# noveens/reviews4rec

Measured on AMD Instinct MI355X. Metric: train ratings/sec, higher is better.
Workload: dtype f32

## Files before the change

### include/r4r.h

```cpp
#ifndef R4R_H
#define R4R_H

#include <stddef.h>
#include <stdint.h>

#ifdef __cplusplus
extern "C" {
#endif

#define R4R_OK 0
#define R4R_ERR_ARG (-1)
#define R4R_ERR_LAUNCH (-2)
#define R4R_ERR_WORKSPACE (-3)

int r4r_version(void);
const char *r4r_last_error(void);

size_t r4r_textcnn_ws_bytes(int64_t N, int T, int E, int F, int64_t V);
int r4r_textcnn_fwd(const float *table, int64_t V, const int64_t *idx,
                    const float *conv_w, const float *conv_b,
                    float *pooled, int32_t *argmax,
                    void *ws, size_t ws_bytes,
                    int64_t N, int T, int E, int F, void *stream);

// ... 64 lines not shown
                       int64_t N, int R, int L, void *stream);

int r4r_mse_fwd_bwd(const float *out, const float *y, float *se, float *g_out,
                    int64_t N, float denom, void *stream);

int r4r_sqdist_mean_fwd(const float *a, const float *b, float *out, int64_t N, int L, void *stream);
int r4r_sqdist_mean_bwd(const float *a, const float *b, const float *g_out, float *g_a, float *g_b,
                        int64_t N, int L, void *stream);

int r4r_adam_chunk_elems(void);
int r4r_adam_multi(int ntensor, const uint64_t *p, const uint64_t *g, const uint64_t *m, const uint64_t *v,
                   const int64_t *numel, float lr, double beta1, double beta2, float eps,
                   float weight_decay, int64_t step, const int64_t *step_dev, void *stream);
int r4r_adam_gathered(float *p, const float *gathered, int world, float *g_sum, float *m, float *v,
                      int64_t numel, float lr, double beta1, double beta2, float eps,
                      float weight_decay, int64_t step, void *stream);
int r4r_adam_gathered_guarded(float *p, const float *gathered, int world, float *g_sum, float *m, float *v,
                              int64_t numel, float lr, double beta1, double beta2, float eps,
                              float weight_decay, int64_t step, const uint32_t *abort_word, void *stream);

int r4r_peer_segment_create(int64_t bytes, void **ptr, uint8_t *handle);
int r4r_peer_segment_open(const uint8_t *handle, void **ptr);
int r4r_peer_segment_close(void *ptr);
int r4r_peer_segment_destroy(void *ptr);
int r4r_peer_push(const float *src, int64_t numel, const uint64_t *peer_dst, const uint64_t *peer_flags,
                  uint32_t *arrive, int rank, int world, uint32_t epoch, const uint32_t *wait_flags,
                  uint32_t *timed_out, double timeout_s, void *stream);
int r4r_peer_wait(const uint32_t *flags, int world, uint32_t epoch, uint32_t *timed_out, double timeout_s, void *stream);


#define R4R_CONV_AUTO 0
#define R4R_CONV_DIRECT 1
#define R4R_CONV_PROJECT 2
int r4r_deepconn_nparam(void);
int r4r_deepconn_layout(int E, int L, int64_t *offsets, int64_t *sizes, int64_t *total);
size_t r4r_deepconn_ws_bytes(int64_t B, int T, int E, int L, int64_t V);
size_t r4r_deepconn_ws_mult_offset(int64_t B, int T, int E, int L, int64_t V);
size_t r4r_deepconn_ws_count_offset(int64_t B, int T, int E, int L, int64_t V, int tower, int buffer);
size_t r4r_deepconn_ws_partials_offset(int64_t B, int T, int E, int L, int64_t V, int tower, int which);
size_t r4r_deepconn_ws_plan_offset(int64_t B, int T, int E, int L, int64_t V, int tower, int buffer, int which);
size_t r4r_deepconn_ws_state_offset(int64_t B, int T, int E, int L, int64_t V, int tower, int buffer, int which);
int r4r_deepconn_step(const float *table, int64_t V, const int64_t *user_idx, const int64_t *item_idx,
                      const float *y, float *flat_p, float *flat_g,
                      float *pred, float *se, float *sse_accum,
                      void *ws, size_t ws_bytes,
                      int64_t B, int T, int E, int L,
                      float dropout_p, int training, uint64_t seed, uint64_t offset,
                      float inv_denom, int conv_algo, int token_buffer, int tokens_ready,
                      const int64_t *next_user_idx, const int64_t *next_item_idx,
                      float *flat_m, float *flat_v, float lr, double beta1, double beta2, float eps,
                      float weight_decay, int64_t adam_step, void *stream);
int r4r_deepconn_tail_fold(int on);
int r4r_deepconn_tail(int64_t B, int E, int L);
int r4r_deepconn_tokens(const int64_t *user_idx, const int64_t *item_idx, void *ws, size_t ws_bytes,
                        int64_t B, int T, int E, int L, int64_t V, int conv_algo, int token_buffer,
                        int discard, void *stream);

#define R4R_TIMING_TEXTCNN_FWD 0
#define R4R_TIMING_TEXTCNN_WGRAD 1
#define R4R_TIMING_ADAM 2
#define R4R_TIMING_PROJ_GEMM 3
#define R4R_TIMING_PROJ_GATHER 4
#define R4R_TIMING_SLOTS 8
int r4r_timing_enable(int slot_mask);
int r4r_timing_read(int slot, double *total_ms, int64_t *count, int reset);

size_t r4r_mf_ws_bytes(int64_t B, int D, int64_t n_users, int64_t n_items);
size_t r4r_mf_ws_persist_bytes(int64_t B, int D, int64_t n_users, int64_t n_items);
size_t r4r_mf_ws_mult_offset(int64_t B, int D, int64_t n_users, int64_t n_items);
size_t r4r_mf_ws_grad_offset(int64_t B, int D, int64_t n_users, int64_t n_items, int which);
int r4r_mf_step(const int64_t *uid, const int64_t *iid, const float *y,
                const uint64_t *p, const uint64_t *m, const uint64_t *v,
                int64_t n_users, int64_t n_items, int D,
                float *pred, float *se, float *sse_accum, void *ws, size_t ws_bytes, int64_t B,
                float dropout_p, int training, uint64_t seed, uint64_t offset, float inv_denom,
                int sweep_period, int64_t sweep_base, int sweep_all,
                float lr, double beta1, double beta2, float eps, float weight_decay, int64_t adam_step,
                void *stream);

int r4r_mf_rows_flush(const uint64_t *p, const uint64_t *m, const uint64_t *v,
                      int64_t n_users, int64_t n_items, int D, void *ws, size_t ws_bytes, int64_t B,
                      int sweep_period, int64_t sweep_base,
                      float lr, double beta1, double beta2, float eps, float weight_decay, int64_t adam_step,
                      void *stream);
size_t r4r_mf_ws_flag_offset(int64_t B, int D, int64_t n_users, int64_t n_items);

int r4r_sse_accumulate(const float *se, int64_t n, float *accum, void *stream);

size_t r4r_mf_dp_block_bytes(int64_t B_pad, int D);
int r4r_mf_grad(const int64_t *uid, const int64_t *iid, const float *y, const uint64_t *p,
                const uint64_t *m, const uint64_t *v,
                int64_t n_users, int64_t n_items, int D, float *pred, float *se, void *block, float *mult,
                int64_t B, int64_t B_pad, float dropout_p, int training, uint64_t seed, uint64_t offset,
                float inv_denom, void *ws, int sweep_period, int64_t sweep_base,
                float lr, double beta1, double beta2, float eps, float weight_decay, int64_t adam_step,
                void *stream);
int r4r_mf_apply(const void *blocks, int world, int64_t B_pad, const uint64_t *p, const uint64_t *m,
                 const uint64_t *v, int64_t n_users, int64_t n_items, int D, void *ws, size_t ws_bytes,
                 int sweep_period, int64_t sweep_base, int sweep_all,
                 const float *se, int64_t se_n, float *sse_accum,
                 float lr, double beta1, double beta2, float eps, float weight_decay, int64_t adam_step,
                 void *stream);
int r4r_mf_grad_push(const int64_t *uid, const int64_t *iid, const float *y, const uint64_t *p,
                     const uint64_t *m, const uint64_t *v,
                     int64_t n_users, int64_t n_items, int D, float *pred, float *se, float *mult,
                     int64_t B, int64_t B_pad, float dropout_p, int training, uint64_t seed, uint64_t offset,
// ... 390 lines not shown
```

### reviews4rec_amd/csrc/engine.hip

```cpp
#include <stdlib.h>

#include "trace_device.h"
#include "textcnn.h"
#include "wgrad_device.h"
#include "tokens_device.h"
#include "adam_device.h"

namespace r4r {

constexpr int F_CONV = 100;
constexpr int FM_K = 8;
constexpr int MAX_L = 128;

enum { P_UCW = 0, P_UCB, P_UFW, P_UFB, P_ICW, P_ICB, P_IFW, P_IFB, P_FMV, P_FMLW, P_FMLB, P_GB, P_COUNT };

struct Layout {
    int64_t off[P_COUNT], size[P_COUNT], total;
};

static Layout make_layout(int E, int L) {
    Layout lay;
    const int64_t sz[P_COUNT] = {(int64_t)F_CONV * 3 * E, F_CONV, (int64_t)L * F_CONV, L,
                                 (int64_t)F_CONV * 3 * E, F_CONV, (int64_t)L * F_CONV, L,
                                 (int64_t)2 * L * FM_K, 2 * L, 1, 1};
    int64_t o = 0;
    for (int i = 0; i < P_COUNT; ++i) {
        lay.off[i] = o;
        lay.size[i] = sz[i];
        o += (sz[i] + 31) & ~(int64_t)31;
    }
    lay.total = o;
    return lay;
}

struct HeadArgs {
    const float *pmax[2]; const int *parg[2];
    const float *fc_w[2]; const float *fc_b[2];
    const float *V, *lin_w, *lin_b, *gbias;
    const float *y;
    float *pooled[2]; int *argmax[2];
    float *g_pooled[2];
    float *mult;
    float *x, *s, *g, *gz;
    float *pred, *se;
    int64_t B;
    int L, tiles, training, want_grad;
    float p_drop, inv_denom;
    uint64_t seed, offset;
    PlanArgs plan;
    int *plan_spent[2];
    TokenArgs marks;
    int mark_wgs;
};


constexpr int HEAD_MAX_TILES = 8;

#define SEL2(arr, s) ((s) ? (arr)[1] : (arr)[0])
HEAD_TRACE_DEFINE(r4r_debug_dc_head_trace)
template <int ML>
__global__ __launch_bounds__(256) void deepconn_head_wg_kernel(HeadArgs a) {
    if ((int64_t)blockIdx.x >= a.B) {
        const int fb = (int)blockIdx.x - (int)a.B, flag_wgs = (2 * a.plan.units + 3) / 4;
        if (fb < flag_wgs) {
            segment_flags_wave(a.plan, fb * 4 + (int)(threadIdx.x >> 6));
        } else {
            const HeadArgs &A = kernel_args<HeadArgs>();
            token_mark_block(A.marks, fb - flag_wgs, A.mark_wgs, 256);
        }
        return;
    }
    HEAD_STAMP(0)
    constexpr int N2 = 2 * ML, PARTS = 256 / N2;
    __shared__ float sw[2][ML][F_CONV + 1];
    __shared__ float sfb[N2], slw[N2], sz[N2];
    __shared__ float sV[N2][FM_K];
    __shared__ float sp[2][F_CONV + 4];
    __shared__ float red[N2][PARTS + 1];
    const int tid = threadIdx.x, lane = tid & 63, w = tid >> 6;
    const int64_t b = blockIdx.x;
    const int L = a.L, n = 2 * L;
    const float lin_b0 = a.lin_b[0], gbias0 = a.gbias[0], yb = a.y ? a.y[b] : 0.f;

    constexpr int FQ = F_CONV / 4;
    typedef float hq4 __attribute__((ext_vector_type(4)));
    constexpr int WREGS = (2 * ML * FQ + 255) / 256;
    hq4 wreg[WREGS];
    const int wtot = 2 * L * FQ;
#pragma unroll
    for (int k = 0; k < WREGS; ++k) {
        const int i = min(tid + 256 * k, wtot - 1);
        const int t = i >= L * FQ;
        wreg[k] = *reinterpret_cast<const hq4 *>(SEL2(a.fc_w, t) + 4 * (i - t * L * FQ));
    }
    const int tn = min(tid, n - 1);
    const float fbreg = SEL2(a.fc_b, tn >= L)[tn - (tn >= L ? L : 0)];
    const float lwreg = a.lin_w[tn];
    constexpr int VREGS = (N2 * FM_K + 255) / 256;
    float vreg[VREGS];
#pragma unroll
    for (int k = 0; k < VREGS; ++k) vreg[k] = a.V[min(tid + 256 * k, n * FM_K - 1)];
    if (b == 0 && tid < 2 && SEL2(a.plan_spent, tid)) SEL2(a.plan_spent, tid)[0] = 0;

    {
        const int t = w >> 1, f = lane + 64 * (w & 1), fc = min(f, F_CONV - 1);
        float best = -INFINITY;
        int bp = -1;
        if (a.tiles <= HEAD_MAX_TILES) {
            float v[HEAD_MAX_TILES];
            int pp[HEAD_MAX_TILES];
#pragma unroll
            for (int k = 0; k < HEAD_MAX_TILES; ++k) {
                const size_t o = ((size_t)b * a.tiles + min(k, a.tiles - 1)) * NP + fc;
                v[k] = SEL2(a.pmax, t)[o];
                pp[k] = SEL2(a.parg, t)[o];
            }
#pragma unroll
            for (int k = 0; k < HEAD_MAX_TILES; ++k)
                if (v[k] > best) { best = v[k]; bp = pp[k]; }
        } else {
            for (int k0 = 0; k0 < a.tiles; k0 += HEAD_MAX_TILES) {
                float v[HEAD_MAX_TILES];
                int pp[HEAD_MAX_TILES];
#pragma unroll
                for (int k = 0; k < HEAD_MAX_TILES; ++k) {
                    const bool in = k0 + k < a.tiles;
                    const size_t o = ((size_t)b * a.tiles + (in ? k0 + k : 0)) * NP + fc;
                    v[k] = in ? SEL2(a.pmax, t)[o] : -INFINITY;
                    pp[k] = SEL2(a.parg, t)[o];
                }
#pragma unroll
                for (int k = 0; k < HEAD_MAX_TILES; ++k)
                    if (v[k] > best) { best = v[k]; bp = pp[k]; }
            }
        }
        if (!(best > 0.f)) { best = 0.f; bp = -1; }
        if (f < F_CONV) {
            sp[t][f] = best;
            SEL2(a.pooled, t)[b * F_CONV + f] = best;
            SEL2(a.argmax, t)[b * F_CONV + f] = bp;
        }
    }
    HEAD_STAMP(1)
#pragma unroll
    for (int k = 0; k < WREGS; ++k) {
        const int i = tid + 256 * k;
        if (i < wtot) {
            const int t = i >= L * FQ, r = i - t * L * FQ, l = r / FQ, f0 = 4 * (r - l * FQ);
#pragma unroll
            for (int c = 0; c < 4; ++c) sw[t][l][f0 + c] = wreg[k][c];
        }
    }
    if (tid < n) { sfb[tid] = fbreg; slw[tid] = lwreg; }
#pragma unroll
    for (int k = 0; k < VREGS; ++k) {
        const int i = tid + 256 * k;
        if (i < n * FM_K) sV[i / FM_K][i % FM_K] = vreg[k];
    }
    __syncthreads();
    HEAD_STAMP(2)

    {
        const int o = tid / PARTS, part = tid - o * PARTS;
        if (o < n) {
            const int t = o / L, l = o - t * L;
            float acc = 0.f;
            for (int f = part; f < F_CONV; f += PARTS) acc = fmaf(sp[t][f], sw[t][l][f], acc);
            red[o][part] = acc;
        }
    }
    __syncthreads();
    const bool has_y = a.y != nullptr, want = has_y && a.want_grad;
    if (w == 0) {
        constexpr int NI = (N2 + 63) / 64;
        float xi[NI], mult[NI], lw[NI], gacc[NI];
#pragma unroll
        for (int u = 0; u < NI; ++u) {
            const int i = lane + 64 * u;
            xi[u] = 0.f; mult[u] = 1.f; gacc[u] = 0.f;
            lw[u] = (i < n) ? slw[i] : 0.f;
            if (i < n) {
                float acc = 0.f;
#pragma unroll
                for (int q = 0; q < PARTS; ++q) acc += red[i][q];
                xi[u] = acc + sfb[i];
            }
            if (a.training && a.p_drop > 0.f && i < n) {
                const uint32_t r = philox_first_word(a.offset + (uint64_t)(b * n + i), a.seed);
                const float uu = (float)(r >> 8) * (1.0f / 16777216.0f);
                mult[u] = (uu >= a.p_drop) ? 1.f / (1.f - a.p_drop) : 0.f;
            }
            xi[u] *= mult[u];
        }
        float inter = 0.f;
        float sk_keep[FM_K];
#pragma unroll
        for (int k = 0; k < FM_K; ++k) {
            float pv = 0.f, pv2 = 0.f, vv[NI];
#pragma unroll
            for (int u = 0; u < NI; ++u) {
                const int i = lane + 64 * u;
                vv[u] = (i < n) ? sV[i][k] : 0.f;
                pv += xi[u] * vv[u];
                pv2 += xi[u] * xi[u] * vv[u] * vv[u];
            }
            const float sk = wave_sum(pv);
            const float s2 = wave_sum(pv2);
            inter += sk * sk - s2;
#pragma unroll
            for (int u = 0; u < NI; ++u) gacc[u] += sk * vv[u] - xi[u] * vv[u] * vv[u];
            sk_keep[k] = sk;
        }
        float pl = 0.f;
#pragma unroll
        for (int u = 0; u < NI; ++u) pl += xi[u] * lw[u];
        const float lin = wave_sum(pl);
        const float pred = (0.5f * inter + lin + lin_b0) + gbias0;
        if (lane == 0) a.pred[b] = pred;
        if (has_y) {
            const float d = pred - yb;
            if (lane == 0) a.se[b] = d * d;
            if (want) {
                const float g = 2.f * d * a.inv_denom;
#pragma unroll
                for (int u = 0; u < NI; ++u) {
                    const int i = lane + 64 * u;
                    const float gx = g * (gacc[u] + lw[u]);
                    const float gz = gx * mult[u];
                    if (i < n) {
                        sz[i] = gz;
                        a.x[b * n + i] = xi[u];
                        a.gz[b * n + i] = gz;
                        a.mult[b * n + i] = mult[u];
                    }
                }
                if (lane < FM_K) {
                    float sv = 0.f;
#pragma unroll
                    for (int k = 0; k < FM_K; ++k) if (lane == k) sv = sk_keep[k];
                    a.s[b * FM_K + lane] = sv;
                }
                if (lane == 0) a.g[b] = g;
            }
        }
    }
    if (!want) return;
    __syncthreads();
    HEAD_STAMP(3)
    if (tid < 2 * F_CONV) {
        const int t = tid >= F_CONV, f = tid - t * F_CONV;
        float acc = 0.f;
        for (int l = 0; l < L; ++l) acc = fmaf(sz[t * L + l], sw[t][l][f], acc);
        SEL2(a.g_pooled, t)[b * F_CONV + f] = acc;
    }
    HEAD_STAMP(4)
}

struct HeadGradArgs {
    const float *pooled[2];
    const float *x, *s, *g, *gz;
    const float *V;
    const float *se;
    float *g_fc_w[2], *g_fc_b[2], *g_V, *g_lin_w, *g_lin_b, *g_gb;
    float *sse_accum;
    int64_t B;
    int L;
};

constexpr int HG_ROWS = 16, HG_COLS = 16;
template <bool STEP = false>
__device__ __forceinline__ void head_grad_block(const HeadGradArgs &a, int blk, const FlatAdam *opt = nullptr) {
    __shared__ float red[HG_ROWS][HG_COLS];
    const int ox = threadIdx.x & (HG_COLS - 1), rg = threadIdx.x / HG_COLS;
    const int L = a.L, n = 2 * L;
    const int n_fcw = L * F_CONV;
    const int seg[9] = {n_fcw, L, n_fcw, L, n * FM_K, n, 1, 1, 1};
    int o = blk * HG_COLS + ox;
    int which = -1, local = 0, acc_o = o;
#pragma unroll
    for (int k = 0; k < 9; ++k) {
        if (which < 0) {
            if (acc_o < seg[k]) { which = k; local = acc_o; }
            else acc_o -= seg[k];
        }
    }
    float P = 0.f, M = 0.f, V = 0.f;
    int po = 0;
    bool stepping = false;
    if constexpr (STEP) {
        if (opt->on && rg == 0 && which >= 0 && which < 8) {
            const float *dst = which == 0 ? a.g_fc_w[0] + local : (which == 1 ? a.g_fc_b[0] + local : (which == 2 ? a.g_fc_w[1] + local :
                  (which == 3 ? a.g_fc_b[1] + local : (which == 4 ? a.g_V + local : (which == 5 ? a.g_lin_w + local :
                  (which == 6 ? a.g_lin_b : a.g_gb))))));
            po = (int)(dst - opt->g);
            stepping = true;
        }
    }
    float s = 0.f;
    if (which >= 0) {
        const bool is_w = which == 0 || which == 2, is_b = which == 1 || which == 3, is_v = which == 4, is_lw = which == 5;
        const int t = which >> 1;
        const int wl = local / F_CONV, wf = local - wl * F_CONV;
        const int vi = local / FM_K, vk = local - vi * FM_K;
        const float *pa = (is_w || is_b) ? a.gz : (which == 8 ? a.se : a.g);
        const int64_t sa = (is_w || is_b) ? n : 1;
        const int64_t oa = is_w ? t * L + wl : (is_b ? t * L + local : 0);
// ... 43 lines not shown
        }
        if constexpr (STEP) {
            if (stepping) {
                adam_elem(P, t, M, V, opt->s);
                opt->p[po] = P; opt->m[po] = M; opt->v[po] = V;
            }
        }
    }
}

BWD_TRACE_DEFINE(r4r_debug_dc_bwd_trace)
struct DcBackwardArgs {
    WgradArgs w;
    HeadGradArgs h;
    int hg_blocks;
    TokenArgs nx;
    PlanArgs plan;
};
__global__ __launch_bounds__(WG_THREADS, 8) void deepconn_backward_kernel(DcBackwardArgs) {
    const DcBackwardArgs &A = kernel_args<DcBackwardArgs>();
    const WgradArgs &w = A.w;
    const HeadGradArgs &h = A.h;
    const TokenArgs &nx = A.nx;
    const PlanArgs &plan = A.plan;
    const int hg_blocks = A.hg_blocks;
    BWD_STAMP(0, wall_clock64())
    BWD_STAMP(2, (unsigned long long)blockIdx.z + 1)
    if (blockIdx.z == 1 || blockIdx.z == 2) {
        wgrad_block(w, blockIdx.x, blockIdx.y, blockIdx.z - 1);
    } else if (blockIdx.z == 0) {
        for (int blk = blockIdx.y * gridDim.x + blockIdx.x; blk < hg_blocks; blk += gridDim.x * gridDim.y) {
            head_grad_block(h, blk);
            __syncthreads();
        }
    } else {
        const int np = plan.units > 0 ? 2 : 0, blk = blockIdx.y * gridDim.x + blockIdx.x;
        if (blk < np) segment_plan_block<WG_THREADS>(plan, blk);
        else token_mark_block(nx, blk - np, gridDim.x * gridDim.y - np, WG_THREADS);
    }
#ifdef R4R_TRACE
    __syncthreads();
#endif
    BWD_STAMP(1, wall_clock64())
}

struct DcFoldArgs {
    WgradArgs w;
    FlatAdam opt;
    HeadGradArgs h;
    int hg_blocks;
    TokenArgs nx;
    PlanArgs plan;
    int comp_blocks;
};
static_assert(WG_THREADS % 64 == 0, "the 256-thread roles of the fold launch are whole waves: the others end before any barrier");
template <bool BIGV>
__global__ __launch_bounds__(WG_ROW_MAX_THREADS, 8) void deepconn_backward_fold_kernel(DcFoldArgs) {
    const DcFoldArgs &A = kernel_args<DcFoldArgs>();
    BWD_STAMP(0, wall_clock64())
    BWD_STAMP(2, (unsigned long long)blockIdx.z + 1)
    if (blockIdx.z == 1 || blockIdx.z == 2) {
        wgrad_row_block(A.w, A.opt, blockIdx.x, blockIdx.y, blockIdx.z - 1);
    } else {
        if (threadIdx.x >= WG_THREADS) return;
        const int blk0 = blockIdx.y * gridDim.x + blockIdx.x, nblk = gridDim.x * gridDim.y;
        if (blockIdx.z == 0) {
            for (int blk = blk0; blk < A.hg_blocks; blk += nblk) {
                head_grad_block<true>(A.h, blk, &A.opt);
                __syncthreads();
            }
        } else {
            const int np = A.plan.units > 0 ? 2 : 0, comp_blocks = A.comp_blocks;
            const int blk = ((int)blockIdx.z - 3) * nblk + blk0;
            if (blk < np) {
                segment_plan_block<WG_THREADS>(A.plan, blk);
            } else if (blk - np < 2 * comp_blocks) {
                const int t = (blk - np) >= comp_blocks;
                const TokenTower &tw = t ? A.nx.t[1] : A.nx.t[0];
                if constexpr (BIGV) token_compact_block<WG_THREADS / 64, COMPACT_BIG_G>(tw, A.nx.V, blk - np - t * comp_blocks);
                else token_compact_block<WG_THREADS / 64, 1>(tw, A.nx.V, blk - np - t * comp_blocks);
            }
        }
    }
#ifdef R4R_TRACE
    __syncthreads();
#endif
    BWD_STAMP(1, wall_clock64())
}

constexpr int RED_THREADS = 256;
struct FusedAdam {
    float *p, *m, *v;
    const float *g;
    int64_t lo[2], hi[2];
    AdamScalars s;
    int on;
};
__global__ __launch_bounds__(RED_THREADS) void deepconn_reduce_kernel(WgradArgs w, int red_blocks, int comp_blocks,
                                                                      TokenArgs nx, FusedAdam opt) {
    const int bx = blockIdx.x;
    if (bx < red_blocks) {
        const WgradTower &tw = w.t[blockIdx.y];
        const int nw = w.F * 3 * w.E;
        const int i = bx * RED_THREADS + threadIdx.x;
        const float *gp0 = i < nw ? tw.d_w + i : (i < nw + w.F ? tw.d_b + (i - nw) : nullptr);
        const int64_t o = gp0 ? gp0 - opt.g : 0;
        float P = 0.f, M = 0.f, V = 0.f;
        if (opt.on && gp0) { P = opt.p[o]; M = opt.m[o]; V = opt.v[o]; }
        float *dst;
        const float g = wgrad_reduce_elem(w, blockIdx.y, i, dst);
        if (opt.on && dst) {
            adam_elem(P, g, M, V, opt.s);
            opt.p[o] = P; opt.m[o] = M; opt.v[o] = V;
        }
    } else if (bx < red_blocks + comp_blocks) {
        token_compact_auto<RED_THREADS / 64>(nx.t[blockIdx.y], nx.V, bx - red_blocks);
    } else {
        const int64_t o = opt.lo[blockIdx.y] + (int64_t)(bx - red_blocks - comp_blocks) * RED_THREADS + threadIdx.x;
        if (o < opt.hi[blockIdx.y]) {
            float P = opt.p[o], M = opt.m[o], V = opt.v[o];
            adam_elem(P, opt.g[o], M, V, opt.s);
            opt.p[o] = P; opt.m[o] = M; opt.v[o] = V;
        }
    }
}

__global__ void sse_only_kernel(const float *__restrict__ se, float *__restrict__ accum, int64_t B) {
    __shared__ float red[256];
    float s = 0.f;
    for (int64_t i = threadIdx.x; i < B; i += 256) s += se[i];
    red[threadIdx.x] = s;
    __syncthreads();
    for (int off = 128; off > 0; off >>= 1) {
        if ((int)threadIdx.x < off) red[threadIdx.x] += red[threadIdx.x + off];
        __syncthreads();
    }
    if (threadIdx.x == 0) accum[0] += red[0];
}

struct StepWs {
    float *wp[2], *pmax[2]; int *parg[2];
    int *flags[2][2], *slot[2][2], *list[2][2], *count[2][2]; float *ptab[2];
    int *live[2][2], *perm[2][2], *plan_ready[2][2];
    float *pooled[2]; int *argmax[2]; float *g_pooled[2];
    float *mult, *x, *s, *g, *gz;
    float *part_w[2], *part_b[2];
    size_t bytes;
};

static StepWs carve(void *ws, int64_t B, int T, int E, int L, int64_t V) {
    StepWs w;
    char *p = static_cast<char *>(ws);
    auto take = [&](size_t nbytes) { char *r = p; p += align256(nbytes); return r; };
    const size_t tiles128 = (size_t)(T + 2 + 127) / 128;
    const int ns = textcnn_wgrad_splits(B);
    for (int t = 0; t < 2; ++t) {
        w.wp[t] = reinterpret_cast<float *>(take(textcnn_wp_floats(E) * 4));
        w.pmax[t] = reinterpret_cast<float *>(take((size_t)B * tiles128 * NP * 4));
        w.parg[t] = reinterpret_cast<int *>(take((size_t)B * tiles128 * NP * 4));
        w.pooled[t] = reinterpret_cast<float *>(take((size_t)B * F_CONV * 4));
        w.argmax[t] = reinterpret_cast<int *>(take((size_t)B * F_CONV * 4));
        w.g_pooled[t] = reinterpret_cast<float *>(take((size_t)B * F_CONV * 4));
        w.part_w[t] = reinterpret_cast<float *>(take((size_t)ns * F_CONV * 3 * E * 4));
        w.part_b[t] = reinterpret_cast<float *>(take((size_t)ns * F_CONV * 4));
        for (int bf = 0; bf < 2; ++bf) {
            w.flags[bf][t] = reinterpret_cast<int *>(take((size_t)(V + 4) * 4));
            w.slot[bf][t] = reinterpret_cast<int *>(take((size_t)(V + 4) * 4));
            w.list[bf][t] = reinterpret_cast<int *>(take((size_t)proj_row_capacity(B, T, V) * 4));
            w.count[bf][t] = reinterpret_cast<int *>(take(256));
        }
        w.ptab[t] = reinterpret_cast<float *>(take(proj_ptab_floats(B, T, V) * 4));
    }
    w.mult = reinterpret_cast<float *>(take((size_t)B * 2 * L * 4));
    w.x = reinterpret_cast<float *>(take((size_t)B * 2 * L * 4));
    w.gz = reinterpret_cast<float *>(take((size_t)B * 2 * L * 4));
    w.s = reinterpret_cast<float *>(take((size_t)B * FM_K * 4));
    w.g = reinterpret_cast<float *>(take((size_t)B * 4));
    for (int t = 0; t < 2; ++t)
        for (int bf = 0; bf < 2; ++bf) {
            w.live[bf][t] = reinterpret_cast<int *>(take((size_t)PLAN_MAX_UNITS * 4));
            w.perm[bf][t] = reinterpret_cast<int *>(take((size_t)PLAN_MAX_UNITS * 4));
            w.plan_ready[bf][t] = reinterpret_cast<int *>(take(256));
        }
    w.bytes = (size_t)(p - static_cast<char *>(ws));
    return w;
}

}

using namespace r4r;

extern "C" int r4r_deepconn_nparam(void) { return P_COUNT; }

extern "C" int r4r_deepconn_layout(int E, int L, int64_t *offsets, int64_t *sizes, int64_t *total) {
    R4R_REQUIRE(E > 0 && L > 0 && L <= MAX_L && offsets && sizes && total, "deepconn_layout: bad arguments");
    const Layout lay = make_layout(E, L);
    for (int i = 0; i < P_COUNT; ++i) { offsets[i] = lay.off[i]; sizes[i] = lay.size[i]; }
    *total = lay.total;
    return R4R_OK;
}

extern "C" size_t r4r_deepconn_ws_bytes(int64_t B, int T, int E, int L, int64_t V) {
    if (B < 0 || T <= 0 || E <= 0 || L <= 0 || V <= 0) return 0;
    return carve(nullptr, B, T, E, L, V).bytes;
}

extern "C" size_t r4r_deepconn_ws_mult_offset(int64_t B, int T, int E, int L, int64_t V) {
    char base[1];
    const StepWs w = carve(base, B, T, E, L, V);
    return (size_t)(reinterpret_cast<char *>(w.mult) - base);
}

extern "C" size_t r4r_deepconn_ws_count_offset(int64_t B, int T, int E, int L, int64_t V, int tower, int buffer) {
    char base[1];
    const StepWs w = carve(base, B, T, E, L, V);
    return (size_t)(reinterpret_cast<char *>(w.count[buffer & 1][tower & 1]) - base);
}

extern "C" size_t r4r_deepconn_ws_partials_offset(int64_t B, int T, int E, int L, int64_t V, int tower, int which) {
    char base[1];
    const StepWs w = carve(base, B, T, E, L, V);
    const void *at = which ? static_cast<const void *>(w.parg[tower & 1]) : w.pmax[tower & 1];
    return (size_t)(static_cast<const char *>(at) - base);
}
extern "C" size_t r4r_deepconn_ws_plan_offset(int64_t B, int T, int E, int L, int64_t V, int tower, int buffer, int which) {
    char base[1];
    const StepWs w = carve(base, B, T, E, L, V);
    const int t = tower & 1, bf = buffer & 1;
    const void *at[3] = {w.perm[bf][t], w.plan_ready[bf][t], w.live[bf][t]};
    return (which < 0 || which > 2) ? 0 : (size_t)(static_cast<const char *>(at[which]) - base);
}

extern "C" size_t r4r_deepconn_ws_state_offset(int64_t B, int T, int E, int L, int64_t V, int tower, int buffer, int which) {
    char base[1];
    const StepWs w = carve(base, B, T, E, L, V);
    const int t = tower & 1, bf = buffer & 1;
    const void *at[4] = {w.flags[bf][t], w.slot[bf][t], w.list[bf][t], w.argmax[t]};
    return (which < 0 || which > 3) ? 0 : (size_t)(static_cast<const char *>(at[which]) - base);
}

static bool plan_applies(int64_t B, int T) {
    const int tiles = proj_tiles(T);
    return proj_gather_plan() && (tiles & 1) == 0 && B * tiles <= PLAN_MAX_UNITS;
}

static int g_tail_fold = -1;
static int tail_fold_switch() {
    if (g_tail_fold < 0) {
        const char *e = getenv("R4R_TAIL");
        g_tail_fold = (e && e[0] == 'o') ? 0 : 1;
    }
    return g_tail_fold;
}
static bool tail_folds(int64_t B, int E, int L) {
    if (!tail_fold_switch() || B < 1 || E <= 0 || E % 4 != 0 || L > 64) return false;
    const int ns = textcnn_wgrad_splits(B);
    return wgrad_row_applies(B, E, ns, (int)cdiv(B, ns));
}
extern "C" int r4r_deepconn_tail_fold(int on) {
    const int before = tail_fold_switch();
    g_tail_fold = on ? 1 : 0;
    return before;
}
extern "C" int r4r_deepconn_tail(int64_t B, int E, int L) { return tail_folds(B, E, L) ? 1 : 0; }

extern "C" int r4r_deepconn_tokens(const int64_t *user_idx, const int64_t *item_idx, void *ws, size_t ws_bytes,
                                   int64_t B, int T, int E, int L, int64_t V, int conv_algo, int token_buffer,
                                   int discard, void *stream) {
    R4R_REQUIRE(user_idx && item_idx && ws, "deepconn_tokens: null pointer");
    R4R_REQUIRE(token_buffer == 0 || token_buffer == 1, "deepconn_tokens: token_buffer must be 0 or 1");
    if (ws_bytes < r4r_deepconn_ws_bytes(B, T, E, L, V)) {
        set_error("deepconn_tokens: workspace %zu < %zu bytes", ws_bytes, r4r_deepconn_ws_bytes(B, T, E, L, V));
        return R4R_ERR_WORKSPACE;
    }
    if (B == 0 || textcnn_pick_algo(conv_algo, B, T, E, F_CONV) != R4R_CONV_PROJECT) return R4R_OK;
    const StepWs w = carve(ws, B, T, E, L, V);
    if (discard) {
        for (int t = 0; t < 2; ++t) {
            (void)hipMemsetAsync(w.count[token_buffer][t], 0, sizeof(int), as_stream(stream));
            (void)hipMemsetAsync(w.plan_ready[token_buffer][t], 0, sizeof(int), as_stream(stream));
        }
        return check_launch("deepconn_tokens(discard)");
    }
    ProjTower pt[2];
    const int64_t *idx[2] = {user_idx, item_idx};
    for (int t = 0; t < 2; ++t) {
        pt[t] = ProjTower{};
        pt[t].idx = idx[t];
        pt[t].flags = w.flags[token_buffer][t]; pt[t].slot = w.slot[token_buffer][t];
        pt[t].list = w.list[token_buffer][t]; pt[t].count = w.count[token_buffer][t];
    }
    return textcnn_proj_tokens_launch(V, pt, 2, B, T, false, as_stream(stream));
}

extern "C" int r4r_deepconn_step(const float *table, int64_t V, const int64_t *user_idx, const int64_t *item_idx,
                                 const float *y, float *flat_p, float *flat_g,
                                 float *pred, float *se, float *sse_accum,
                                 void *ws, size_t ws_bytes,
                                 int64_t B, int T, int E, int L,
                                 float dropout_p, int training, uint64_t seed, uint64_t offset,
                                 float inv_denom, int conv_algo, int token_buffer, int tokens_ready,
                                 const int64_t *next_user_idx, const int64_t *next_item_idx,
                                 float *flat_m, float *flat_v, float lr, double beta1, double beta2, float eps,
                                 float weight_decay, int64_t adam_step,
                                 void *stream) {
    R4R_REQUIRE(table && user_idx && item_idx && flat_p && pred && ws, "deepconn_step: null pointer");
    R4R_REQUIRE(!flat_m == !flat_v, "deepconn_step: flat_m and flat_v go together");
    R4R_REQUIRE(!flat_m || (flat_g && adam_step >= 1), "deepconn_step: the fused optimiser needs gradients and "
                                                       "adam_step >= 1");
    R4R_REQUIRE(!next_user_idx == !next_item_idx, "deepconn_step: next_user_idx and next_item_idx go together");
    R4R_REQUIRE(!next_user_idx || flat_g, "deepconn_step: the next batch's tokens ride on the backward launches "
                                          "(training steps only)");
    R4R_REQUIRE(V > 0 && B >= 0 && T > 0, "deepconn_step: bad sizes");
    R4R_REQUIRE(E > 0 && E % 4 == 0, "deepconn_step: word_embed_size %d must be a positive multiple of 4", E);
    R4R_REQUIRE(L > 0 && L <= MAX_L, "deepconn_step: latent_size %d outside 1..%d", L, MAX_L);
    R4R_REQUIRE(!flat_g || (y && se), "deepconn_step: gradients need ratings y and the se buffer");
    R4R_REQUIRE(!y || se, "deepconn_step: se buffer required when y is given");
// ... 38 lines not shown
    } else {
        FwdTower ft[2];
        for (int t = 0; t < 2; ++t) {
            ft[t].idx = idx[t];
            ft[t].conv_w = P[t ? P_ICW : P_UCW];
            ft[t].conv_b = P[t ? P_ICB : P_UCB];
            ft[t].wp = w.wp[t]; ft[t].pmax = w.pmax[t]; ft[t].parg = w.parg[t];
        }
        if (int rc = textcnn_fwd_launch(table, ft, 2, B, T, E, F_CONV, st)) return rc;
        tiles = textcnn_tiles(T);
    }

    HeadArgs h;
    for (int t = 0; t < 2; ++t) {
        h.pmax[t] = w.pmax[t]; h.parg[t] = w.parg[t];
        h.fc_w[t] = P[t ? P_IFW : P_UFW]; h.fc_b[t] = P[t ? P_IFB : P_UFB];
        h.pooled[t] = w.pooled[t]; h.argmax[t] = w.argmax[t]; h.g_pooled[t] = w.g_pooled[t];
    }
    h.V = P[P_FMV]; h.lin_w = P[P_FMLW]; h.lin_b = P[P_FMLB]; h.gbias = P[P_GB];
    h.y = y; h.mult = w.mult; h.x = w.x; h.s = w.s; h.g = w.g; h.gz = w.gz;
    h.pred = pred; h.se = se;
    h.B = B; h.L = L; h.tiles = tiles; h.training = training; h.want_grad = flat_g != nullptr;
    h.p_drop = dropout_p; h.inv_denom = inv_denom; h.seed = seed; h.offset = offset;
    const bool planning = next_user_idx && flat_g && algo == R4R_CONV_PROJECT && plan_applies(B, T);
    PlanArgs plan{};
    if (planning) {
        const int ob = token_buffer ^ 1;
        plan.idx[0] = next_user_idx; plan.idx[1] = next_item_idx;
        for (int t = 0; t < 2; ++t) {
            plan.live[t] = w.live[ob][t]; plan.perm[t] = w.perm[ob][t]; plan.plan_ready[t] = w.plan_ready[ob][t];
        }
        plan.T = T; plan.tiles = proj_tiles(T); plan.units = (int)(B * plan.tiles);
    }
    h.plan = plan;
    for (int t = 0; t < 2; ++t) h.plan_spent[t] = algo == R4R_CONV_PROJECT ? w.plan_ready[token_buffer][t] : nullptr;
    const bool fold = flat_g && tail_folds(B, E, L);
    const bool prefetch = next_user_idx && algo == R4R_CONV_PROJECT;
    TokenArgs nx{};
    if (prefetch) {
        ProjTower nt[2];
        const int64_t *nidx[2] = {next_user_idx, next_item_idx};
        const int ob = token_buffer ^ 1;
        for (int t = 0; t < 2; ++t) {
            nt[t] = ProjTower{};
            nt[t].idx = nidx[t];
            nt[t].flags = w.flags[ob][t]; nt[t].slot = w.slot[ob][t];
            nt[t].list = w.list[ob][t]; nt[t].count = w.count[ob][t];
        }
        nx = make_token_args(V, nt, 2, B, T);
    }
    h.marks = nx;
    const int64_t mark_want = cdiv(B * (int64_t)T, 256);
    h.mark_wgs = (fold && prefetch) ? (int)(mark_want < 1024 ? mark_want : 1024) : 0;
    const unsigned head_wgs = (unsigned)B + (unsigned)cdiv(2 * (int64_t)plan.units, 4) + (unsigned)h.mark_wgs;
    if (L <= 16) deepconn_head_wg_kernel<16><<<head_wgs, 256, 0, st>>>(h);
    else if (L <= 32) deepconn_head_wg_kernel<32><<<head_wgs, 256, 0, st>>>(h);
    else if (L <= 64) deepconn_head_wg_kernel<64><<<head_wgs, 256, 0, st>>>(h);
    else deepconn_head_wg_kernel<128><<<head_wgs, 256, 0, st>>>(h);

    if (!flat_g) {
        if (y && sse_accum) sse_only_kernel<<<1, 256, 0, st>>>(se, sse_accum, B);
        return check_launch("deepconn_step(forward)");
    }

    HeadGradArgs hg;
    for (int t = 0; t < 2; ++t) {
        hg.pooled[t] = w.pooled[t];
        hg.g_fc_w[t] = G[t ? P_IFW : P_UFW]; hg.g_fc_b[t] = G[t ? P_IFB : P_UFB];
    }
    hg.x = w.x; hg.s = w.s; hg.g = w.g; hg.gz = w.gz; hg.V = P[P_FMV]; hg.se = se;
    hg.g_V = G[P_FMV]; hg.g_lin_w = G[P_FMLW]; hg.g_lin_b = G[P_FMLB]; hg.g_gb = G[P_GB];
    hg.sse_accum = sse_accum; hg.B = B; hg.L = L;
    const int nout = 2 * (L * F_CONV + L) + 2 * L * FM_K + 2 * L + 3;
    const int hg_blocks = (nout + HG_COLS - 1) / HG_COLS;

    WgradTower wt[2];
    WgradArgs wa;
    for (int t = 0; t < 2; ++t) {
        wt[t].idx = idx[t]; wt[t].g_pooled = w.g_pooled[t]; wt[t].argmax = w.argmax[t];
        wt[t].part_w = w.part_w[t]; wt[t].part_b = w.part_b[t];
        wt[t].d_w = G[t ? P_ICW : P_UCW]; wt[t].d_b = G[t ? P_ICB : P_UCB];
    }
    for (int k = 0; k < MAX_TOWERS; ++k) wa.t[k] = wt[k < 2 ? k : 0];
    wa.table = table; wa.N = B; wa.T = T; wa.E = E; wa.F = F_CONV;
    wa.table_bytes = (int64_t)V * E * 4;
    wa.nsplit = textcnn_wgrad_splits(B);
    wa.per_split = (int)cdiv(B, wa.nsplit);
    const int comp_blocks = prefetch ? (int)cdiv((V + 3) / 4, RED_THREADS * compact_groups(V)) : 0;
    if (fold) {
        FlatAdam fo{};
        if (flat_m) {
            fo.on = 1;
            fo.p = flat_p; fo.m = flat_m; fo.v = flat_v; fo.g = flat_g;
            fo.s = adam_make_scalars(lr, beta1, beta2, eps, weight_decay, adam_step, nullptr);
        }
        const int side = prefetch ? (planning ? 2 : 0) + 2 * comp_blocks : 0;
        const unsigned nz = 3 + (unsigned)cdiv(side, F_CONV * 3);
        {
            ScopedTiming tm(R4R_TIMING_TEXTCNN_WGRAD, st);
            const DcFoldArgs fa{wa, fo, hg, hg_blocks, nx, plan, comp_blocks};
            const dim3 grid(F_CONV, 3, nz);
            const int nthr = wgrad_row_threads(E, wa.nsplit);
            if (V > COMPACT_BIG_V) deepconn_backward_fold_kernel<true><<<grid, nthr, 0, st>>>(fa);
            else deepconn_backward_fold_kernel<false><<<grid, nthr, 0, st>>>(fa);
        }
        return check_launch("deepconn_step");
    }
    {
        ScopedTiming tm(R4R_TIMING_TEXTCNN_WGRAD, st);
        deepconn_backward_kernel<<<dim3(F_CONV, wa.nsplit, prefetch ? 4 : 3), WG_THREADS, 0, st>>>(DcBackwardArgs{wa, hg, hg_blocks, nx, plan});
    }
    const int red_blocks = (F_CONV * 3 * E + F_CONV + RED_THREADS - 1) / RED_THREADS;
    FusedAdam opt{};
    int opt_blocks = 0;
    if (flat_m) {
        opt.on = 1;
        opt.p = flat_p; opt.m = flat_m; opt.v = flat_v; opt.g = flat_g;
        opt.lo[0] = lay.off[P_UFW]; opt.hi[0] = lay.off[P_ICW];
        opt.lo[1] = lay.off[P_IFW]; opt.hi[1] = lay.total;
        opt.s = adam_make_scalars(lr, beta1, beta2, eps, weight_decay, adam_step, nullptr);
        const int64_t longest = opt.hi[0] - opt.lo[0] > opt.hi[1] - opt.lo[1] ? opt.hi[0] - opt.lo[0] : opt.hi[1] - opt.lo[1];
        opt_blocks = (int)cdiv(longest, RED_THREADS);
    }
    deepconn_reduce_kernel<<<dim3(red_blocks + comp_blocks + opt_blocks, 2), RED_THREADS, 0, st>>>(
        wa, red_blocks, comp_blocks, nx, opt);
    return check_launch("deepconn_step");
}

extern "C" int r4r_sse_accumulate(const float *se, int64_t n, float *accum, void *stream) {
    R4R_REQUIRE(accum && (se || n == 0) && n >= 0, "sse_accumulate: bad arguments");
    if (n == 0) return R4R_OK;
    sse_only_kernel<<<1, 256, 0, as_stream(stream)>>>(se, accum, n);
    return check_launch("sse_accumulate");
}
```

### reviews4rec_amd/csrc/wgrad_device.h

```cpp
#pragma once
#include "adam_device.h"
#include "textcnn.h"

namespace r4r {

typedef float wg_f32x4 __attribute__((ext_vector_type(4)));

constexpr int WG_THREADS = 256;

struct WgradArgs {
    WgradTower t[MAX_TOWERS];
    const float *table;
    int64_t N;
    int T, E, F, per_split, nsplit;
    int64_t table_bytes = 0;
};

constexpr int WG_CHUNK = 16;
constexpr int WG_FLIGHT = 8;

template <bool FIRST>
__device__ __forceinline__ void wgrad_block_pass(const WgradArgs &a, int f, int s, int tower, int v0,
                                                 long (&s_off)[WG_CHUNK][3], float (&s_g)[WG_CHUNK]) {
    const WgradTower &tw = a.t[tower];
    const float *__restrict__ table = a.table;
    const int64_t *__restrict__ idx = tw.idx;
    const float *__restrict__ gp = tw.g_pooled;
    const int *__restrict__ argmax = tw.argmax;
    const int T = a.T, E = a.E, F = a.F;
    const int64_t n0 = (int64_t)s * a.per_split;
    const int64_t n1 = min(a.N, n0 + (int64_t)a.per_split);
    const int nvec = 3 * E / 4;
    const int tid = threadIdx.x;
    wg_f32x4 acc[2] = {(wg_f32x4){0.f, 0.f, 0.f, 0.f}, (wg_f32x4){0.f, 0.f, 0.f, 0.f}};
    int vj[2], ve[2];
#pragma unroll
    for (int k = 0; k < 2; ++k) {
        const int v = v0 + tid + k * WG_THREADS;
        vj[k] = (v * 4) / E;
        ve[k] = v * 4 - vj[k] * E;
    }
    float sb = 0.f;
    const bool buf_ok = a.table_bytes > 0 && a.table_bytes < (1ll << 32);
    const __amdgpu_buffer_rsrc_t rsrc = __builtin_amdgcn_make_buffer_rsrc(const_cast<float *>(table), 0, buf_ok ? (int)(unsigned)a.table_bytes : 0, 0x00020000);
    for (int64_t c0 = n0; c0 < n1; c0 += WG_CHUNK) {
        const int nd = (int)min((int64_t)WG_CHUNK, n1 - c0);
        __syncthreads();
        if (tid < nd * 3) {
            const int d = tid / 3, j = tid - d * 3;
            const int64_t n = c0 + d;
            const int p = argmax[n * F + f];
            const float gv = gp[n * F + f];
            const int t = p - 2 + j;
            long off = -1;
            if (p >= 0 && t >= 0 && t < T) off = (long)idx[n * T + t] * E;
            s_off[d][j] = off;
            if (j == 0) s_g[d] = (p >= 0) ? gv : 0.f;
        }
        __syncthreads();
// ... 121 lines not shown
                    v[d] = *reinterpret_cast<const wg_f32x4 *>(table + (off < 0 ? 0 : off) + ve);
                }
#pragma unroll
                for (int d = 0; d < WG_CHUNK; ++d) {
                    const wg_f32x4 sum = acc + p_g[wave][r0 + d] * v[d];
                    acc = p_off[wave][r0 + d][vj] >= 0 ? sum : acc;
                }
            }
        }
        if (live && lane == 0)
            for (int d = 0; d < nd; ++d) sb += p_g[wave][d];
    }
    if (live && lane < nvec) *reinterpret_cast<wg_f32x4 *>(tw.part_w + ((size_t)s * F + f) * 3 * E + lane * 4) = acc;
    if (live && lane == 0) tw.part_b[(size_t)s * F + f] = sb;
}

constexpr int WG_MAX_SPLITS = 16;

__device__ __forceinline__ float wgrad_reduce_elem(const WgradArgs &a, int tower, int i, float *&dst) {
    const WgradTower &tw = a.t[tower];
    const int nw = a.F * 3 * a.E;
    const float *src;
    size_t stride;
    if (i < nw) { src = tw.part_w + i; stride = (size_t)nw; dst = tw.d_w + i; }
    else if (i < nw + a.F) { src = tw.part_b + (i - nw); stride = (size_t)a.F; dst = tw.d_b + (i - nw); }
    else { dst = nullptr; return 0.f; }
    float v[WG_MAX_SPLITS];
#pragma unroll
    for (int k = 0; k < WG_MAX_SPLITS; ++k) v[k] = src[(size_t)(k < a.nsplit ? k : 0) * stride];
    float s = 0.f;
#pragma unroll
    for (int k = 0; k < WG_MAX_SPLITS; ++k)
        if (k < a.nsplit) s += v[k];
    *dst = s;
    return s;
}

__device__ __forceinline__ void wgrad_reduce_block(const WgradArgs &a, int tower, int blk) {
    float *dst;
    (void)wgrad_reduce_elem(a, tower, blk * (int)blockDim.x + (int)threadIdx.x, dst);
}

constexpr int WG_ROW_MAX_THREADS = 1024;
constexpr int WG_ROW_MAX_DOCS = WG_MAX_SPLITS * WG_CHUNK;
constexpr unsigned WG_ROW_NONE = 0xffffffffu;
inline bool wgrad_row_applies(int64_t N, int E, int nsplit, int per_split) {
    return N >= 1 && N <= WG_ROW_MAX_DOCS && per_split <= WG_CHUNK && nsplit <= WG_MAX_SPLITS && E % 4 == 0 &&
           (int64_t)nsplit * (E / 4) <= WG_ROW_MAX_THREADS;
}
inline int wgrad_row_threads(int E, int nsplit) {
    const int t = (nsplit * (E / 4) + 63) & ~63;
    return t < WG_THREADS ? WG_THREADS : t;
}
__device__ __forceinline__ void wgrad_row_block(const WgradArgs &a, const FlatAdam &opt, int f, int tap, int tower) {
    __shared__ long r_off[WG_ROW_MAX_DOCS];
    __shared__ unsigned r_bo[WG_ROW_MAX_DOCS];
    __shared__ float r_g[WG_ROW_MAX_DOCS];
    __shared__ __attribute__((aligned(16))) float r_part[4 * WG_ROW_MAX_THREADS];
    __shared__ float r_sb[WG_MAX_SPLITS];
    const WgradTower &tw = a.t[tower];
    const float *__restrict__ table = a.table;
    const int T = a.T, E = a.E, F = a.F, e4 = E / 4, nsplit = a.nsplit;
    const int N = (int)a.N;
    const int tid = threadIdx.x;
    const int s = tid / e4, c = tid - s * e4, ve = 4 * c;
    const bool worker = s < nsplit;
    const int tot = E + (tap == 0 ? 1 : 0);
    float *const row_w = tw.d_w + ((size_t)f * 3 + tap) * E;
    float *const dst0 = tid < E ? row_w + tid : tw.d_b + f;
    float P = 0.f, M = 0.f, V = 0.f;
    if (opt.on && tid < tot) {
        const int o = (int)(dst0 - opt.g);
        P = opt.p[o]; M = opt.m[o]; V = opt.v[o];
    }
    if (tid < N) {
        const int p = tw.argmax[(int64_t)tid * F + f];
        const float gv = tw.g_pooled[(int64_t)tid * F + f];
        const int t = p - 2 + tap;
        long off = -1;
        if (p >= 0 && t >= 0 && t < T) off = (long)tw.idx[(int64_t)tid * T + t] * E;
        r_off[tid] = off;
        r_bo[tid] = off >= 0 ? (unsigned)(off * 4) : WG_ROW_NONE;
        r_g[tid] = (p >= 0) ? gv : 0.f;
    }
    __syncthreads();
    const int n0 = worker ? s * a.per_split : 0;
    const int nd = worker ? max(0, min(N, n0 + a.per_split) - n0) : 0;
    wg_f32x4 acc = {0.f, 0.f, 0.f, 0.f};
    const bool buf_ok = a.table_bytes > 0 && a.table_bytes < (1ll << 32);
    const __amdgpu_buffer_rsrc_t rsrc = __builtin_amdgcn_make_buffer_rsrc(const_cast<float *>(table), 0, buf_ok ? (int)(unsigned)a.table_bytes : 0, 0x00020000);
    if (worker && nd > 0) {
        if (buf_ok) {
#pragma unroll
            for (int d0 = 0; d0 < WG_CHUNK; d0 += WG_FLIGHT) {
                wg_f32x4 row[WG_FLIGHT];
                bool on[WG_FLIGHT];
#pragma unroll
                for (int u = 0; u < WG_FLIGHT; ++u) {
                    const int d = d0 + u;
                    const unsigned rv = r_bo[n0 + d];
                    const unsigned ro = d < nd ? rv : WG_ROW_NONE;
                    on[u] = ro != WG_ROW_NONE;
                    const unsigned bo = on[u] ? ro + (unsigned)(ve * 4) : 0xfffffff0u;
                    row[u] = __builtin_bit_cast(wg_f32x4, __builtin_amdgcn_raw_buffer_load_b128(rsrc, (int)bo, 0, 0));
                }
#pragma unroll
                for (int u = 0; u < WG_FLIGHT; ++u) {
                    const wg_f32x4 sum = acc + r_g[n0 + d0 + u] * row[u];
                    acc = on[u] ? sum : acc;
                }
                __builtin_amdgcn_sched_barrier(0);
            }
        } else {
#pragma unroll 4
            for (int d = 0; d < nd; ++d) {
                const long off = r_off[n0 + d];
                if (off >= 0) acc += r_g[n0 + d] * *reinterpret_cast<const wg_f32x4 *>(table + off + ve);
            }
        }
    }
    r_part[4 * tid] = acc.x; r_part[4 * tid + 1] = acc.y; r_part[4 * tid + 2] = acc.z; r_part[4 * tid + 3] = acc.w;
    if (tap == 0 && tid < nsplit) {
        const int b0 = tid * a.per_split, bn = max(0, min(N, b0 + a.per_split) - b0);
        float sb = 0.f;
        for (int d = 0; d < bn; ++d) sb += r_g[b0 + d];
        r_sb[tid] = sb;
    }
    __syncthreads();
// ... 19 lines not shown
```

Baseline: 1.439 million.

## Hand off precomputed token byte offsets and grads from head to wgrad kernel

```diff
diff --git a/include/r4r.h b/include/r4r.h
--- a/include/r4r.h
+++ b/include/r4r.h
@@ -140,6 +140,8 @@
                       float weight_decay, int64_t adam_step, void *stream);
 int r4r_deepconn_tail_fold(int on);
 int r4r_deepconn_tail(int64_t B, int E, int L);
+int r4r_deepconn_handoff(int on);
+size_t r4r_deepconn_ws_handoff_offset(int64_t B, int T, int E, int L, int64_t V, int tower);
 int r4r_deepconn_tokens(const int64_t *user_idx, const int64_t *item_idx, void *ws, size_t ws_bytes,
                         int64_t B, int T, int E, int L, int64_t V, int conv_algo, int token_buffer,
                         int discard, void *stream);
diff --git a/reviews4rec_amd/csrc/engine.hip b/reviews4rec_amd/csrc/engine.hip
--- a/reviews4rec_amd/csrc/engine.hip
+++ b/reviews4rec_amd/csrc/engine.hip
@@ -51,6 +51,9 @@
     int *plan_spent[2];
     TokenArgs marks;
     int mark_wgs;
+    const int64_t *idx[2];
+    unsigned *row_bo[2];
+    int T, E;
 };
 
 
@@ -102,8 +105,10 @@
     for (int k = 0; k < VREGS; ++k) vreg[k] = a.V[min(tid + 256 * k, n * FM_K - 1)];
     if (b == 0 && tid < 2 && SEL2(a.plan_spent, tid)) SEL2(a.plan_spent, tid)[0] = 0;
 
+    const int pf_t = w >> 1, pf_f = lane + 64 * (w & 1);
+    int pf_bp;
     {
-        const int t = w >> 1, f = lane + 64 * (w & 1), fc = min(f, F_CONV - 1);
+        const int t = pf_t, f = pf_f, fc = min(f, F_CONV - 1);
         float best = -INFINITY;
         int bp = -1;
         if (a.tiles <= HEAD_MAX_TILES) {
@@ -135,6 +140,7 @@
             }
         }
         if (!(best > 0.f)) { best = 0.f; bp = -1; }
+        pf_bp = bp;
         if (f < F_CONV) {
             sp[t][f] = best;
             SEL2(a.pooled, t)[b * F_CONV + f] = best;
@@ -159,6 +165,12 @@
     }
     __syncthreads();
     HEAD_STAMP(2)
+    int64_t pf_id[3];
+    {
+        const int64_t *ids = SEL2(a.idx, pf_t) + b * a.T;
+#pragma unroll
+        for (int j = 0; j < 3; ++j) pf_id[j] = ids[min(max(pf_bp - 2 + j, 0), a.T - 1)];
+    }
 
     {
         const int o = tid / PARTS, part = tid - o * PARTS;
@@ -247,11 +259,22 @@
     if (!want) return;
     __syncthreads();
     HEAD_STAMP(3)
-    if (tid < 2 * F_CONV) {
-        const int t = tid >= F_CONV, f = tid - t * F_CONV;
+    if (pf_f < F_CONV) {
+        const int t = pf_t, f = pf_f;
         float acc = 0.f;
         for (int l = 0; l < L; ++l) acc = fmaf(sz[t * L + l], sw[t][l][f], acc);
         SEL2(a.g_pooled, t)[b * F_CONV + f] = acc;
+        if (a.row_bo[0]) {
+            wg_u32x4 rec;
+#pragma unroll
+            for (int j = 0; j < 3; ++j) {
+                const int p = pf_bp - 2 + j;
+                const long off = (long)pf_id[j] * a.E;
+                rec[j] = (pf_bp >= 0 && p >= 0 && p < a.T && off >= 0) ? (unsigned)(off * 4) : WG_ROW_NONE;
+            }
+            rec[3] = __float_as_uint(pf_bp >= 0 ? acc : 0.f);
+            reinterpret_cast<wg_u32x4 *>(SEL2(a.row_bo, t))[b * F_CONV + f] = rec;
+        }
     }
     HEAD_STAMP(4)
 }
@@ -401,6 +424,7 @@
     TokenArgs nx;
     PlanArgs plan;
     int comp_blocks;
+    const unsigned *row_bo[2];
 };
 static_assert(WG_THREADS % 64 == 0, "the 256-thread roles of the fold launch are whole waves: the others end before any barrier");
 template <bool BIGV>
@@ -409,7 +433,8 @@
     BWD_STAMP(0, wall_clock64())
     BWD_STAMP(2, (unsigned long long)blockIdx.z + 1)
     if (blockIdx.z == 1 || blockIdx.z == 2) {
-        wgrad_row_block(A.w, A.opt, blockIdx.x, blockIdx.y, blockIdx.z - 1);
+        const int t = blockIdx.z - 1;
+        wgrad_row_block(A.w, A.opt, blockIdx.x, blockIdx.y, t, SEL2(A.row_bo, t));
     } else {
         if (threadIdx.x >= WG_THREADS) return;
         const int blk0 = blockIdx.y * gridDim.x + blockIdx.x, nblk = gridDim.x * gridDim.y;
@@ -494,6 +519,7 @@
     float *pooled[2]; int *argmax[2]; float *g_pooled[2];
     float *mult, *x, *s, *g, *gz;
     float *part_w[2], *part_b[2];
+    unsigned *row_bo[2];
     size_t bytes;
 };
 
@@ -531,6 +557,8 @@
             w.perm[bf][t] = reinterpret_cast<int *>(take((size_t)PLAN_MAX_UNITS * 4));
             w.plan_ready[bf][t] = reinterpret_cast<int *>(take(256));
         }
+    for (int t = 0; t < 2; ++t)
+        w.row_bo[t] = reinterpret_cast<unsigned *>(take((size_t)B * F_CONV * 16));
     w.bytes = (size_t)(p - static_cast<char *>(ws));
     return w;
 }
@@ -612,6 +640,25 @@
     return before;
 }
 extern "C" int r4r_deepconn_tail(int64_t B, int E, int L) { return tail_folds(B, E, L) ? 1 : 0; }
+
+static int g_handoff = -1;
+static int handoff_switch() {
+    if (g_handoff < 0) {
+        const char *e = getenv("R4R_HANDOFF");
+        g_handoff = (e && e[0] == '0') ? 0 : 1;
+    }
+    return g_handoff;
+}
+extern "C" int r4r_deepconn_handoff(int on) {
+    const int before = handoff_switch();
+    g_handoff = on ? 1 : 0;
+    return before;
+}
+extern "C" size_t r4r_deepconn_ws_handoff_offset(int64_t B, int T, int E, int L, int64_t V, int tower) {
+    char base[1];
+    const StepWs w = carve(base, B, T, E, L, V);
+    return (size_t)(reinterpret_cast<const char *>(w.row_bo[tower & 1]) - base);
+}
 
 extern "C" int r4r_deepconn_tokens(const int64_t *user_idx, const int64_t *item_idx, void *ws, size_t ws_bytes,
                                    int64_t B, int T, int E, int L, int64_t V, int conv_algo, int token_buffer,
@@ -756,6 +803,12 @@
     h.marks = nx;
     const int64_t mark_want = cdiv(B * (int64_t)T, 256);
     h.mark_wgs = (fold && prefetch) ? (int)(mark_want < 1024 ? mark_want : 1024) : 0;
+    const bool handoff = fold && handoff_switch() && (int64_t)V * E * 4 < (1ll << 32);
+    for (int t = 0; t < 2; ++t) {
+        h.idx[t] = idx[t];
+        h.row_bo[t] = handoff ? w.row_bo[t] : nullptr;
+    }
+    h.T = T; h.E = E;
     const unsigned head_wgs = (unsigned)B + (unsigned)cdiv(2 * (int64_t)plan.units, 4) + (unsigned)h.mark_wgs;
     if (L <= 16) deepconn_head_wg_kernel<16><<<head_wgs, 256, 0, st>>>(h);
     else if (L <= 32) deepconn_head_wg_kernel<32><<<head_wgs, 256, 0, st>>>(h);
@@ -802,7 +855,8 @@
         const unsigned nz = 3 + (unsigned)cdiv(side, F_CONV * 3);
         {
             ScopedTiming tm(R4R_TIMING_TEXTCNN_WGRAD, st);
-            const DcFoldArgs fa{wa, fo, hg, hg_blocks, nx, plan, comp_blocks};
+            const DcFoldArgs fa{wa, fo, hg, hg_blocks, nx, plan, comp_blocks,
+                                {h.row_bo[0], h.row_bo[1]}};
             const dim3 grid(F_CONV, 3, nz);
             const int nthr = wgrad_row_threads(E, wa.nsplit);
             if (V > COMPACT_BIG_V) deepconn_backward_fold_kernel<true><<<grid, nthr, 0, st>>>(fa);
diff --git a/reviews4rec_amd/csrc/wgrad_device.h b/reviews4rec_amd/csrc/wgrad_device.h
--- a/reviews4rec_amd/csrc/wgrad_device.h
+++ b/reviews4rec_amd/csrc/wgrad_device.h
@@ -5,6 +5,7 @@
 namespace r4r {
 
 typedef float wg_f32x4 __attribute__((ext_vector_type(4)));
+typedef unsigned wg_u32x4 __attribute__((ext_vector_type(4)));
 
 constexpr int WG_THREADS = 256;
 
@@ -232,7 +233,8 @@
     const int t = (nsplit * (E / 4) + 63) & ~63;
     return t < WG_THREADS ? WG_THREADS : t;
 }
-__device__ __forceinline__ void wgrad_row_block(const WgradArgs &a, const FlatAdam &opt, int f, int tap, int tower) {
+__device__ __forceinline__ void wgrad_row_block(const WgradArgs &a, const FlatAdam &opt, int f, int tap, int tower,
+                                                const unsigned *__restrict__ row_bo = nullptr) {
     __shared__ long r_off[WG_ROW_MAX_DOCS];
     __shared__ unsigned r_bo[WG_ROW_MAX_DOCS];
     __shared__ float r_g[WG_ROW_MAX_DOCS];
@@ -253,7 +255,13 @@
         const int o = (int)(dst0 - opt.g);
         P = opt.p[o]; M = opt.m[o]; V = opt.v[o];
     }
-    if (tid < N) {
+    if (row_bo) {
+        if (tid < N) {
+            const wg_u32x4 rec = reinterpret_cast<const wg_u32x4 *>(row_bo)[(int64_t)tid * F + f];
+            r_bo[tid] = tap == 0 ? rec[0] : (tap == 1 ? rec[1] : rec[2]);
+            r_g[tid] = __uint_as_float(rec[3]);
+        }
+    } else if (tid < N) {
         const int p = tw.argmax[(int64_t)tid * F + f];
         const float gv = tw.g_pooled[(int64_t)tid * F + f];
         const int t = p - 2 + tap;
```

Result: no change. 1.451 million (median of 6 runs) (+0.8%).
